# semihkacmaz/CoNFiLD

Measured on AMD Instinct MI355X. Metric: generated fields/sec (256-step sample + CNF decode), Case4 latent, 1/2/4/8 GPU, higher is better.
Workload: dtype f32

## Files before the change

### confild_amd/csrc/unet_kernels.hip

```cpp
#include <algorithm>
#include <cstdlib>

#include "unet_kernels.hpp"

namespace cfd {

__global__ __launch_bounds__(256) void gn_partial_kernel(GnArgs a) {
    const int chunk = blockIdx.x;
    const int64_t b = blockIdx.y;
    const int Ctot = a.Ctot, cq = Ctot / 4, cpg = Ctot / 32;
    const int HW = a.HW;
    const int p0 = (int)((int64_t)HW * chunk / a.nchunks), p1 = (int)((int64_t)HW * (chunk + 1) / a.nchunks);
    const int rows = 256 / cq;
    const int q = threadIdx.x % cq, r0 = threadIdx.x / cq;
    __shared__ double red[2][1024];
    if (r0 < rows) {
        double s[4] = {0, 0, 0, 0}, s2[4] = {0, 0, 0, 0};
        const int c0 = 4 * q;
        for (int p = p0 + r0; p < p1; p += rows) {
            const int64_t pix = b * HW + p;
            const f4 v = c0 < a.C1 ? *(const f4*)(a.src1 + pix * a.C1 + c0)
                                   : *(const f4*)(a.src2 + pix * a.C2 + (c0 - a.C1));
#pragma unroll
            for (int j = 0; j < 4; ++j) {
// ... 1311 lines not shown
            __builtin_amdgcn_global_load_lds((const void*)(src + lane),
                                             (__attribute__((address_space(3))) void*)&ring[stage][piece * 64], 16, 0, 0);
        }
    };
    const int nall = T32 / 32, per = (nall + kcs - 1) / kcs;
    const int blk0 = kc_i * per, nblk = min(per, nall - blk0);
#pragma unroll
    for (int i = 0; i < NS - 1; ++i)
        if (i < nblk) issue(32 * (blk0 + i), i);

    h8v qh[NJ], ql[NJ];
    {
        const int tq = min(q0 + li, T - 1);
#pragma unroll
        for (int j = 0; j < NJ; ++j) {
            const float* qp = base + (int64_t)tq * C3 + 32 * j + 8 * g;
            float v[8];
#pragma unroll
            for (int t = 0; t < 8; ++t) v[t] = qp[t] * a.scale;
            split8_f16(v, qh[j], ql[j]);
        }
    }
    f4 O[ND];
#pragma unroll
    for (int d = 0; d < ND; ++d) O[d] = f4{0.f, 0.f, 0.f, 0.f};
    float mrun = -INFINITY, lrun = 0.f;

    for (int ib = 0; ib < nblk; ++ib) {
        const int kb = 32 * (blk0 + ib), stage = ib % NS;
        if (NS == 3 && ib + 1 < nblk)
            __builtin_amdgcn_s_waitcnt(vmcnt_wait(PPW));
        else
            __builtin_amdgcn_s_waitcnt(vmcnt_wait(0));
        __builtin_amdgcn_s_barrier();
        if (ib + NS - 1 < nblk) issue(kb + 32 * (NS - 1), (ib + NS - 1) % NS);
        if (!active) continue;
        const h8v* kl8 = &ring[stage][lane];
        f4 st[2];
#pragma unroll
        for (int u = 0; u < 2; ++u) {
            st[u] = f4{0.f, 0.f, 0.f, 0.f};
#pragma unroll
            for (int j = 0; j < NJ; ++j) {
                const h8v kh = kl8[((u * NJ + j) * 2) * 64], kl = kl8[((u * NJ + j) * 2 + 1) * 64];
                st[u] = __builtin_amdgcn_mfma_f32_16x16x32_f16(kl, qh[j], st[u], 0, 0, 0);
                st[u] = __builtin_amdgcn_mfma_f32_16x16x32_f16(kh, ql[j], st[u], 0, 0, 0);
                st[u] = __builtin_amdgcn_mfma_f32_16x16x32_f16(kh, qh[j], st[u], 0, 0, 0);
            }
        }
        float mx = -INFINITY;
        if (kb + 32 > T) {
#pragma unroll
            for (int u = 0; u < 2; ++u)
#pragma unroll
                for (int r = 0; r < 4; ++r)
                    if (kb + 16 * u + 4 * g + r >= T) st[u][r] = -INFINITY;
        }
#pragma unroll
        for (int u = 0; u < 2; ++u)
#pragma unroll
            for (int r = 0; r < 4; ++r) mx = fmaxf(mx, st[u][r]);
        mx = fmaxf(mx, __shfl_xor(mx, 16));
        mx = fmaxf(mx, __shfl_xor(mx, 32));
        const float mnew = fmaxf(mrun, mx);
        const float alpha = __builtin_amdgcn_exp2f(mrun - mnew);
        float p[8], ps = 0.f;
#pragma unroll
        for (int u = 0; u < 2; ++u)
#pragma unroll
            for (int r = 0; r < 4; ++r) {
                p[4 * u + r] = __builtin_amdgcn_exp2f(st[u][r] - mnew);
                ps += p[4 * u + r];
            }
        ps += __shfl_xor(ps, 16);
        ps += __shfl_xor(ps, 32);
        lrun = lrun * alpha + ps;
        mrun = mnew;
#pragma unroll
        for (int d = 0; d < ND; ++d) O[d] = O[d] * alpha;
        h8v ph, pl;
        split8_f16(p, ph, pl);
        const h8v* vl8 = &ring[stage][KP * 64 + lane];
#pragma unroll
        for (int d = 0; d < ND; ++d) {
            const h8v vh = vl8[(2 * d) * 64], vl = vl8[(2 * d + 1) * 64];
            O[d] = __builtin_amdgcn_mfma_f32_16x16x32_f16(vl, ph, O[d], 0, 0, 0);
            O[d] = __builtin_amdgcn_mfma_f32_16x16x32_f16(vh, pl, O[d], 0, 0, 0);
            O[d] = __builtin_amdgcn_mfma_f32_16x16x32_f16(vh, ph, O[d], 0, 0, 0);
        }
    }
    if (!active) return;
    const int tq = q0 + li;
    if constexpr (SPLIT) {
        if (tq < T) {
            const int64_t row = ((int64_t)kc_i * (gridDim.z / kcs) + b) * heads + h;
            float* op = a.part + (row * T + tq) * CH;
#pragma unroll
            for (int d = 0; d < ND; ++d) *(f4*)(op + 16 * d + 4 * g) = O[d];
            if (g == 0) {
                float* ml = a.part + (int64_t)kcs * (gridDim.z / kcs) * heads * T * CH;
                *(float2*)(ml + 2 * (row * T + tq)) = float2{mrun, lrun};
            }
        }
        return;
    }
    if (a.lse && g == 0 && tq < T)
        a.lse[((int64_t)b * gridDim.y + h) * T + tq] = (mrun + log2f(lrun)) * 0.69314718055994530942f;
    if (tq < T) {
        float* op = a.out + (b * (int64_t)T + tq) * a.C + (int64_t)h * CH;
        const float inv = 1.0f / lrun;
#pragma unroll
        for (int d = 0; d < ND; ++d) {
            f4 v = O[d] * inv;
            *(f4*)(op + 16 * d + 4 * g) = v;
        }
    }
}

template <int CH>
__global__ __launch_bounds__(256) void attn_combine_kernel(AttnArgs a, int heads, int B) {
    constexpr int Q = CH / 4;
    const int64_t i = (int64_t)blockIdx.x * blockDim.x + threadIdx.x;
    const int64_t rows = (int64_t)B * heads * a.T;
    if (i >= rows * Q) return;
    const int d4 = (int)(i % Q);
    const int64_t r = i / Q;
    const int kc = a.kc;
    const float* ml = a.part + (int64_t)kc * rows * CH;
    float M = -INFINITY;
    for (int c = 0; c < kc; ++c) M = fmaxf(M, ml[2 * (c * rows + r)]);
    float L = 0.f;
    f4 o = {0.f, 0.f, 0.f, 0.f};
    for (int c = 0; c < kc; ++c) {
        const float w = __builtin_amdgcn_exp2f(ml[2 * (c * rows + r)] - M);
        L += w * ml[2 * (c * rows + r) + 1];
        o += w * *(const f4*)(a.part + (c * rows + r) * CH + 4 * d4);
    }
    const int tq = (int)(r % a.T);
    const int64_t bh = r / a.T;
    const int h = (int)(bh % heads);
    const int64_t b = bh / heads;
    *(f4*)(a.out + (b * (int64_t)a.T + tq) * a.C + (int64_t)h * CH + 4 * d4) = o * (1.0f / L);
    if (a.lse && d4 == 0) a.lse[bh * a.T + tq] = (M + log2f(L)) * 0.69314718055994530942f;
}

__global__ void temb_kernel(const int64_t* __restrict__ t, const float* __restrict__ freqs, float* __restrict__ out,
                            int dim) {
    const int b = blockIdx.x;
    const int half = dim / 2;
    const float tf = (float)t[b];
    for (int i = threadIdx.x; i < dim; i += blockDim.x) {
        float v = 0.f;
        if (i < half) {
            v = cosf(tf * freqs[i]);
        } else if (i < 2 * half) {
            v = sinf(tf * freqs[i - half]);
        }
        out[(int64_t)b * dim + i] = v;
    }
}

template <int KW>
__global__ __launch_bounds__(256) void linear_kernel(const float* __restrict__ x, const float* __restrict__ W,
                                                     const float* __restrict__ bias, float* __restrict__ y, int B,
                                                     int K, int N, int act) {
    constexpr int BC = 8;
    extern __shared__ __attribute__((aligned(16))) float xs[];
    const int lane = threadIdx.x & 63;
    const int n = blockIdx.x * 4 + (threadIdx.x >> 6);
    const bool live = n < N;
    CFD_DASSERT(K <= 256 * KW && K % 4 == 0);
    f4 w[KW];
#pragma unroll
    for (int i = 0; i < KW; ++i) {
        const int k = 4 * (lane + 64 * i);
        w[i] = live && k < K ? *(const f4*)(W + (int64_t)n * K + k) : f4{0.f, 0.f, 0.f, 0.f};
    }
    const float bn = live ? bias[n] : 0.f;
    for (int b0 = 0; b0 < B; b0 += BC) {
        const int nb = min(BC, B - b0);
        __syncthreads();
        for (int i = threadIdx.x; i < nb * K; i += 256) {
            const float v = x[(int64_t)b0 * K + i];
            xs[i] = act ? silu_f(v) : v;
        }
        __syncthreads();
        if (!live) continue;
        for (int bb = 0; bb < nb; ++bb) {
            float s = 0.f;
#pragma unroll
            for (int i = 0; i < KW; ++i) {
                const int k = 4 * (lane + 64 * i);
                if (k < K) {
                    const f4 v = *(const f4*)(xs + bb * K + k);
                    s = fmaf(w[i][0], v[0], s);
                    s = fmaf(w[i][1], v[1], s);
                    s = fmaf(w[i][2], v[2], s);
                    s = fmaf(w[i][3], v[3], s);
                }
            }
            for (int o = 32; o > 0; o >>= 1) s += __shfl_xor(s, o);
            if (lane == 0) y[(int64_t)(b0 + bb) * N + n] = s + bn;
        }
    }
}

int gn_chunks(int HW) {
    const int64_t small = std::min<int64_t>(64, HW / 16);
    return (int)std::max<int64_t>(1, std::min<int64_t>(kGnMaxChunks, std::max<int64_t>(HW / 64, small)));
}

static unsigned long long* g_stamps = nullptr;
void stamps_set(unsigned long long* buf) { g_stamps = buf; }
unsigned long long* stamps_buf() { return g_stamps; }
static int g_seq = 0;

static int env_int(const char* name, int dflt) {
    const char* e = getenv(name);
    return e ? atoi(e) : dflt;
}

bool gn2_applies(const GnArgs& a) {
    const int pb = a.plan_b > 0 ? a.plan_b : 8;
    return (int64_t)a.HW * 8 >= (int64_t)4096 * pb && a.Ctot % 4 == 0 && a.C1 % 4 == 0 && a.C2 % 4 == 0 &&
           a.Ctot <= 1024;
}

static int gn_reg_ipt(const GnArgs& a) {
    return a.Ctot % 128 == 0 ? (int)ceil_div(a.HW, 512 / (a.Ctot / 128)) : 0;
}

bool gn_takes_splitk(const GnArgs& a, int B) {
    (void)B;
    if (gn2_applies(a)) return a.C1 % 4 == 0;
    if (a.Ctot % 128 != 0 || a.C1 % 4 != 0) return false;
    return gn_reg_ipt(a) <= 16;
}

void launch_gn(const GnArgs& a0, int B, hipStream_t st) {
    CFD_REQUIRE(a0.Ctot % 32 == 0 && a0.C1 % 4 == 0 && a0.C2 % 4 == 0 && a0.Ctot <= 1024, CFD_ESHAPE,
                "GroupNorm32 needs channels % 32 == 0 (<= 1024)");
    GnArgs a = a0;
    a.nchunks = gn_chunks(a.HW);
    a.B = B;
    a.stamps = g_stamps;
    a.seq = g_seq++;
    CFD_REQUIRE(!a.kpart || gn_takes_splitk(a, B), CFD_ESTATE, "internal: split-K source on a GroupNorm path without it");
    if (gn2_applies(a)) {
        CFD_REQUIRE(!a.kpart || a.kx, CFD_ESTATE, "internal: gn2 needs the split-K sum's destination");
        a.nchunks = gn2_chunks(a.HW, a.plan_b);
        if (gn2_threads(a.nchunks) == 1024) {
            hipLaunchKernelGGL(gn2_stats_kernel<1024>, dim3(a.nchunks, B), dim3(1024), 0, st, a);
            check_launch("gn2_stats_kernel");
            hipLaunchKernelGGL(gn2_apply_kernel<1024>, dim3(a.nchunks, B), dim3(1024), 0, st, a);
        } else {
            hipLaunchKernelGGL(gn2_stats_kernel<256>, dim3(a.nchunks, B), dim3(256), 0, st, a);
            check_launch("gn2_stats_kernel");
            hipLaunchKernelGGL(gn2_apply_kernel<256>, dim3(a.nchunks, B), dim3(256), 0, st, a);
        }
        check_launch("gn2_apply_kernel");
        return;
    }
    const int ipt = gn_reg_ipt(a);
    if (ipt > 0 && ipt <= 32) {
        const dim3 grid((unsigned)(32 * B));
        const int nq = a.Ctot / 128, r256 = 256 / nq, i256 = (a.HW + r256 - 1) / r256;
        if (i256 <= 4) {
            if (i256 <= 1)
                hipLaunchKernelGGL((gn_fused_reg_kernel<1, 256>), grid, dim3(256), 0, st, a);
            else if (i256 <= 2)
                hipLaunchKernelGGL((gn_fused_reg_kernel<2, 256>), grid, dim3(256), 0, st, a);
            else
                hipLaunchKernelGGL((gn_fused_reg_kernel<4, 256>), grid, dim3(256), 0, st, a);
            check_launch("gn_fused_reg_kernel");
            return;
        }
        if (ipt <= 4)
            hipLaunchKernelGGL((gn_fused_reg_kernel<2, 1024>), grid, dim3(1024), 0, st, a);
        else if (ipt <= 8)
            hipLaunchKernelGGL((gn_fused_reg_kernel<4, 1024>), grid, dim3(1024), 0, st, a);
        else if (ipt <= 16)
            hipLaunchKernelGGL((gn_fused_reg_kernel<8, 1024>), grid, dim3(1024), 0, st, a);
        else
            hipLaunchKernelGGL(gn_fused_reg_kernel<32>, grid, dim3(512), 0, st, a);
        check_launch("gn_fused_reg_kernel");
        return;
    }
    hipLaunchKernelGGL(gn_partial_kernel, dim3(a.nchunks, B), dim3(256), 0, st, a);
    check_launch("gn_partial_kernel");
    hipLaunchKernelGGL(gn_finalize_kernel, dim3(B), dim3(1024), 0, st, a);
    check_launch("gn_finalize_kernel");
    const int64_t nq = (int64_t)B * a.HW * a.Ctot / 4;
    hipLaunchKernelGGL(gn_apply_kernel, dim3((unsigned)std::min<int64_t>(4096, ceil_div(nq, 256))), dim3(256), 0, st, a);
    check_launch("gn_apply_kernel");
}


static int even_splits(int nch, int splits) {
    if (splits <= 1) return 1;
    const int per = (nch + splits - 1) / splits;
    return (nch + per - 1) / per;
}

ConvPlan plan_conv(const ConvArgs& a, size_t part_cap_floats) {
    const int plan_b = a.plan_b > 0 ? a.plan_b : 8;
    ConvPlan p;
    const int64_t mn = (int64_t)plan_b * a.Hout * a.Wout;
    p.bn = a.Cout >= 128 ? 128 : 64;
    auto tiles = [&](int bm) { return ceil_div(mn, bm) * ceil_div(a.Cout, p.bn); };
    p.bm = 64;
    int wg_per_tile = 1;
    if (p.bn == 128) {
        p.bm = 128;
        p.nw = 8;
        wg_per_tile = 2;
    }
    const int nkt = a.K / 32;
    p.splits = 1;
    while (tiles(p.bm) * wg_per_tile * p.splits < 768 && nkt / (p.splits * 2) >= 4 && p.splits < 16)
        p.splits *= 2;
    if (a.ks == 1 && !a.tmode && tiles(p.bm) >= 128) p.splits = 1;
    while (p.splits > 1 && (size_t)p.splits * mn * a.Cout > part_cap_floats) p.splits /= 2;
    if (a.wlo && a.ks == 3 && a.stride == 1 && !a.tmode && a.Ctot <= 128 && (int64_t)a.Hout * a.Wout >= 36864)
        return p;
    const int64_t srows = mn / ((int64_t)a.Hout * a.Wout) * a.Hin * a.Win;
    const bool fits32 = srows < (1 << 23) && srows * std::max(a.C1, a.C2) * 4 < (1ll << 30) &&
                        (int64_t)a.Cout * a.K * 2 < (1ll << 31);
    auto halo_splits = [&](int64_t t) {
        const int nch = a.Ctot / 32;
        int sp = 1;
        while (t * sp < 256 && sp * 2 <= nch && sp < 16) sp *= 2;
        while (sp > 1 && (size_t)sp * mn * a.Cout > part_cap_floats) sp /= 2;
        return even_splits(nch, sp);
    };
    if (a.wbf && !a.wlo && !a.tmode && a.ks == 3 && a.stride == 1 && a.Cout >= 128 && fits32 && conv_h_tw(a) > 0) {
        ConvPlan q;
        q.kx = 22;
        q.bm = 256;
        q.bn = 128;
        q.nw = 8;
        q.splits = halo_splits(ceil_div(mn, 256) * ceil_div(a.Cout, 128));
        return q;
    }
    if (a.wbf && a.wlo && !a.tmode && a.ks == 3 && a.stride == 1 && a.Cout >= 128 && fits32) {
        ConvPlan q;
        if (conv_h_tw(a) > 0) {
            q.kx = 20;
            q.bm = 256;
            q.bn = 128;
            q.nw = 8;
            q.splits = halo_splits(ceil_div(mn, 256) * ceil_div(a.Cout, 128));
            return q;
        }
        q.kx = mn >= 2048 ? 2 : 1;
        q.bm = q.kx == 2 ? 256 : 128;
        q.bn = 128;
        q.nw = q.kx == 2 ? 8 : 4;
        const int64_t t = ceil_div(mn, q.bm) * ceil_div(a.Cout, q.bn);
        q.splits = 1;
        while (t * q.splits < 256 && nkt / (q.splits * 2) >= 4 && q.splits < 32) q.splits *= 2;
        while (q.splits > 1 && (size_t)q.splits * mn * a.Cout > part_cap_floats) q.splits /= 2;
        return q;
    }
    return p;
}

int smalln_below() {
    const int v = env_int("CFD_CONV_SMALLN", 1);
    return v == 1 ? 128 : std::max(v, 0);
}

template <bool TMODE, int MODE, bool BUFA>
static void launch_conv_tiles_(const ConvArgs& a, const ConvPlan& p, dim3 grid, hipStream_t st) {
    if constexpr (MODE != 0 && BUFA) {
        static const int smalln = smalln_below();
        if (!TMODE && p.nw == 8 && p.bm == 128 && p.bn == 128 && (int64_t)grid.x * grid.y * grid.z < smalln &&
            a.Cout % 64 == 0) {
            const dim3 g64(grid.x, (unsigned)ceil_div(a.Cout, 64), grid.z);
            hipLaunchKernelGGL((conv_gemm_kernel<128, 64, false, MODE, 8, true>), g64, dim3(512), 0, st, a);
            return;
        }
        if (p.nw == 8 && p.bm == 128 && p.bn == 128 && p.pf == 2) {
            hipLaunchKernelGGL((conv_gemm_kernel<128, 128, TMODE, MODE, 8, true, 2>), grid, dim3(512), 0, st, a);
            return;
        }
        if (p.nw == 8 && p.bm == 128 && p.bn == 128 && p.pf == 3) {
            hipLaunchKernelGGL((conv_gemm_kernel<128, 128, TMODE, MODE, 8, true, 3>), grid, dim3(512), 0, st, a);
            return;
        }
    }
    if (p.nw == 8 && p.bm == 128 && p.bn == 128)
        hipLaunchKernelGGL((conv_gemm_kernel<128, 128, TMODE, MODE, 8, BUFA>), grid, dim3(512), 0, st, a);
    else if (p.bm == 128 && p.bn == 128)
        hipLaunchKernelGGL((conv_gemm_kernel<128, 128, TMODE, MODE, 4, BUFA>), grid, dim3(256), 0, st, a);
    else if (p.bm == 64 && p.bn == 128)
        hipLaunchKernelGGL((conv_gemm_kernel<64, 128, TMODE, MODE, 4, BUFA>), grid, dim3(256), 0, st, a);
    else if (p.bm == 128 && p.bn == 64)
        hipLaunchKernelGGL((conv_gemm_kernel<128, 64, TMODE, MODE, 4, BUFA>), grid, dim3(256), 0, st, a);
    else
        hipLaunchKernelGGL((conv_gemm_kernel<64, 64, TMODE, MODE, 4, BUFA>), grid, dim3(256), 0, st, a);
}

template <bool TMODE, int MODE>
static void launch_conv_tiles(const ConvArgs& a, const ConvPlan& p, dim3 grid, hipStream_t st) {
    if (a.bufaddr) return launch_conv_tiles_<TMODE, MODE, true>(a, p, grid, st);
    launch_conv_tiles_<TMODE, MODE, false>(a, p, grid, st);
}

void launch_splitk_reduce(const ConvArgs& a, int splits, hipStream_t st) {
    const int64_t total4 = (int64_t)a.M * a.Cout / 4;
    hipLaunchKernelGGL(splitk_reduce_kernel, dim3((unsigned)ceil_div(total4, 256)), dim3(256), 0, st, a, splits);
    check_launch("splitk_reduce_kernel");
}

static bool conv_x_falls_back(const ConvArgs& a) {
    static const int force_k1s = env_int("CFD_CONV_FORCE_K1S", 0);
    const int64_t srows = (int64_t)a.Hin * a.Win * (a.M / (a.Hout * a.Wout));
    return force_k1s || !(srows < (1 << 24) && a.M < (1 << 24) && srows * std::max(a.C1, a.C2) * 4 < (1ll << 31));
}

bool conv_runs_k1hb(const ConvArgs& a, const ConvPlan& p) { return p.kx == 22 && !conv_x_falls_back(a); }

bool conv_kv_pack_ok(const ConvArgs& a, const ConvPlan& p, int T) {
    static const int ldsepi = env_int("CFD_CONV_LDSEPI", 1);
    return ldsepi && p.kx < 0 && p.splits == 1 && a.wbf && !a.tmode && a.ks == 1 && a.bias &&
           !a.emb && !a.res && a.Cout % 8 == 0 && a.emb_stride % 4 == 0 && T % 32 == 0 && a.M % T == 0;
}

int launch_conv(const ConvArgs& a, const ConvPlan& p0, hipStream_t st, bool defer) {
    ConvPlan p = p0;
    if (p.kx >= 0 && conv_x_falls_back(a)) {
        p.kx = -1;
        p.bm = p.bn = 128;
        p.nw = 8;
    }
    CFD_REQUIRE(!a.src_bf16 || p.kx == 22, CFD_ESTATE, "internal: a bf16 convolution source needs the K1hb kernel");
    static const int pf = env_int("CFD_CONV_PF", 2);
    if (p.kx < 0) p.pf = pf >= 1 && pf <= 3 ? pf : 1;
    CFD_REQUIRE(a.Ctot % 32 == 0 && a.C1 % 4 == 0 && a.C2 % 4 == 0, CFD_ESHAPE, "conv_gemm needs channels % 32 == 0");
    CFD_REQUIRE(a.K == a.ks * a.ks * a.Ctot, CFD_ESHAPE, "conv K mismatch");
    CFD_REQUIRE(p.splits == 1 || (a.part && a.Cout % 4 == 0), CFD_ESTATE, "split-K needs a partial buffer");
    CFD_REQUIRE(!a.tmode || ((a.stride == 1 || a.stride == 2) && !a.up), CFD_ESHAPE, "transposed conv: stride 1|2");
    const dim3 grid((unsigned)ceil_div(a.M, p.bm), (unsigned)ceil_div(a.Cout, p.bn), p.splits);
    CFD_REQUIRE(!(a.tmode && a.wbf && !a.wlo), CFD_ESTATE, "bf16 input-gradient convolutions are not built");
    static const int xcd = env_int("CFD_CONV_XCD", 4);
    static const int ldsepi = env_int("CFD_CONV_LDSEPI", 1);
    ConvArgs b = a;
    b.stamps = g_stamps;
    b.seq = g_seq++;
    b.ldsepi = ldsepi && a.Cout % 4 == 0 && a.emb_stride % 4 == 0;
    const int xo = xcd == 4 ? (a.wbf && !a.wlo ? 1 : 3) : xcd;
    b.xcd = xo == 3 ? ((int64_t)a.Hout * a.Wout <= 256 ? 2 : 1) : xo < 0 || xo > 2 ? 1 : xo;
    {
        const int64_t srows = (int64_t)a.Hin * a.Win * (a.M / (a.Hout * a.Wout));
        const int64_t wes = (a.wbf || a.wlo) ? 2 : 4;
        b.bufaddr = a.ks * a.ks <= 9 && srows < (1 << 24) && a.M < (1 << 24) &&
                    srows * std::max(a.C1, a.C2) * 4 < (1ll << 31) && (int64_t)a.Cout * a.K * wes < (1ll << 31);
    }
    const ConvArgs& a_ = b;
    if (p.kx >= 0) {
        launch_conv_x(a_, p.kx, p.splits, st);
        if (p.splits > 1 && !defer) launch_splitk_reduce(a, p.splits, st);
        return p.splits;
    }
    if (a.tmode && a.wlo)
        launch_conv_tiles<true, 2>(a_, p, grid, st);
    else if (a.tmode)
        launch_conv_tiles<true, 0>(a_, p, grid, st);
    else if (a.wbf && a.wlo)
        launch_conv_tiles<false, 2>(a_, p, grid, st);
    else if (a.wbf)
        launch_conv_tiles<false, 1>(a_, p, grid, st);
    else
        launch_conv_tiles<false, 0>(a_, p, grid, st);
    check_launch("conv_gemm_kernel");
    if (p.splits > 1 && !defer) launch_splitk_reduce(a, p.splits, st);
    return p.splits;
}

void launch_conv_in(const ConvArgs& a, hipStream_t st) {
    if (a.Cout % 4 == 0 && a.C1 <= 4 && (size_t)9 * a.C1 * a.Cout * 4 <= 64 * 1024) {
        const int64_t n = (int64_t)a.M * (a.Cout / 4);
        hipLaunchKernelGGL(conv_in_vec_kernel, dim3((unsigned)std::min<int64_t>(2048, ceil_div(n, 256))), dim3(256),
                           sizeof(float) * 9 * a.C1 * a.Cout, st, a);
        check_launch("conv_in_vec_kernel");
        return;
    }
    const int64_t n = (int64_t)a.M * a.Cout;
    hipLaunchKernelGGL(conv_in_kernel, dim3((unsigned)ceil_div(n, 256)), dim3(256), 0, st, a);
    check_launch("conv_in_kernel");
}

void launch_conv_out(const ConvArgs& a, hipStream_t st) {
    CFD_REQUIRE(a.Cout <= 4, CFD_ESHAPE, "out_channels must be <= 4");
    const int LP = a.Ctot / 4;
    if (a.Ctot % 4 == 0 && a.C1 == a.Ctot && LP >= 1 && LP <= 64 && (LP & (LP - 1)) == 0 &&
        (size_t)a.Cout * a.K * 4 <= 64 * 1024) {
        const int64_t waves = ceil_div(a.M, 64 / LP);
        hipLaunchKernelGGL(conv_out_vec_kernel, dim3((unsigned)std::min<int64_t>(8192, ceil_div(waves, 4))), dim3(256),
                           sizeof(float) * a.Cout * a.K, st, a, LP);
        check_launch("conv_out_vec_kernel");
        return;
    }
    hipLaunchKernelGGL(conv_out_kernel, dim3((unsigned)ceil_div(a.M, 4)), dim3(256), 0, st, a);
    check_launch("conv_out_kernel");
}

void launch_attention(const AttnArgs& a, int CH, int heads, int B, hipStream_t st) {
    const dim3 grid((unsigned)ceil_div(a.T, 64), heads, B);
    switch (CH) {
        case 16: hipLaunchKernelGGL(attention_kernel<16>, grid, dim3(256), 0, st, a); break;
        case 32: hipLaunchKernelGGL(attention_kernel<32>, grid, dim3(256), 0, st, a); break;
        case 64: hipLaunchKernelGGL(attention_kernel<64>, grid, dim3(256), 0, st, a); break;
        case 128: hipLaunchKernelGGL(attention_kernel<128>, grid, dim3(256), 0, st, a); break;
        default: throw Error{CFD_ESHAPE, "attention head channels must be 16, 32, 64 or 128"};
    }
    check_launch("attention_kernel");
}

size_t attention_split_floats(int T, int C) { return (size_t)(T + 31) / 32 * 32 * C * 2; }

int64_t attention_split_voff(int T, int CH, int heads, int B) {
    const int T32 = (T + 31) / 32 * 32;
    return (int64_t)B * heads * (T32 / 16) * (CH / 32) * 128;
}

int attention_kv_chunks(int T, int heads, int plan_b) {
    const int nblk = (T + 31) / 32;
    const int64_t wgs = (int64_t)plan_b * heads * ceil_div(T, 64);
    int kc = 1;
    while (kc * 4 <= nblk && wgs * kc * 2 <= 256) kc *= 2;
    return kc;
}

size_t attention_part_floats(int T, int C, int CH, int plan_b) {
    const int heads = C / CH, kc = attention_kv_chunks(T, heads, plan_b);
    return kc == 1 ? 0 : (size_t)kc * T * (C + 2 * heads);
}

void launch_attention_split(const AttnArgs& a, int CH, int heads, int B, int plan_b, float* kvws, hipStream_t st,
                            bool packed) {
    CFD_REQUIRE(CH == 32 || CH == 64 || CH == 128, CFD_ESHAPE, "split attention needs head channels 32, 64 or 128");
    const int T32 = (a.T + 31) / 32 * 32;
    h8v* kf = (h8v*)kvws;
    h8v* vf = kf + attention_split_voff(a.T, CH, heads, B);
    if (!packed) {
        const int64_t slots = (int64_t)B * heads * ((T32 / 16) * (CH / 32) * 64 + (T32 / 32) * (CH / 16) * 64);
        hipLaunchKernelGGL(attn_kv_split_kernel, dim3((unsigned)ceil_div(slots, 256)), dim3(256), 0, st, a, CH, heads,
                           B, kf, vf);
        check_launch("attn_kv_split_kernel");
    }
    const int kc = attention_kv_chunks(a.T, heads, plan_b);
    if (kc > 1) {
        CFD_REQUIRE(a.part, CFD_ESTATE, "internal: key-chunked attention without a partial buffer");
        AttnArgs a2 = a;
        a2.kc = kc;
        a2.xcdmap = 0;
        const dim3 grid((unsigned)ceil_div(a.T, 64), heads, B * kc);
        switch (CH) {
            case 32: hipLaunchKernelGGL((attention_dma_kernel<32, 4, 3, true>), grid, dim3(256), 0, st, a2, kf, vf); break;
            case 64: hipLaunchKernelGGL((attention_dma_kernel<64, 4, 3, true>), grid, dim3(256), 0, st, a2, kf, vf); break;
            default: hipLaunchKernelGGL((attention_dma_kernel<128, 4, 3, true>), grid, dim3(256), 0, st, a2, kf, vf); break;
        }
        check_launch("attention_dma_kernel (key chunks)");
        const int64_t n = (int64_t)B * heads * a.T * (CH / 4);
        const dim3 g2((unsigned)ceil_div(n, 256));
        switch (CH) {
            case 32: hipLaunchKernelGGL(attn_combine_kernel<32>, g2, dim3(256), 0, st, a2, heads, B); break;
            case 64: hipLaunchKernelGGL(attn_combine_kernel<64>, g2, dim3(256), 0, st, a2, heads, B); break;
            default: hipLaunchKernelGGL(attn_combine_kernel<128>, g2, dim3(256), 0, st, a2, heads, B); break;
        }
        check_launch("attn_combine_kernel");
        return;
    }
    static const int xcdmap = env_int("CFD_ATTN_XCD", 1);
    AttnArgs a2 = a;
    a2.xcdmap = xcdmap && (heads * B) % 8 == 0 ? 1 : 0;
    const int w8 = a.T >= 512 && (int64_t)B * heads * ceil_div(a.T, 128) >= 256;
    const dim3 grid((unsigned)ceil_div(a.T, w8 ? 128 : 64), heads, B);
    const dim3 blk(w8 ? 512 : 256);
    switch (CH * 2 + w8) {
        case 64: hipLaunchKernelGGL((attention_dma_kernel<32, 4>), grid, blk, 0, st, a2, kf, vf); break;
        case 65: hipLaunchKernelGGL((attention_dma_kernel<32, 8>), grid, blk, 0, st, a2, kf, vf); break;
        case 128: hipLaunchKernelGGL((attention_dma_kernel<64, 4>), grid, blk, 0, st, a2, kf, vf); break;
        case 129: hipLaunchKernelGGL((attention_dma_kernel<64, 8>), grid, blk, 0, st, a2, kf, vf); break;
        case 256: hipLaunchKernelGGL((attention_dma_kernel<128, 4>), grid, blk, 0, st, a2, kf, vf); break;
        default: hipLaunchKernelGGL((attention_dma_kernel<128, 8>), grid, blk, 0, st, a2, kf, vf); break;
    }
    check_launch("attention_dma_kernel");
}

void launch_temb(const int64_t* t, const float* freqs, float* out, int dim, int B, hipStream_t st) {
    hipLaunchKernelGGL(temb_kernel, dim3(B), dim3(128), 0, st, t, freqs, out, dim);
    check_launch("temb_kernel");
}

void launch_linear(const float* x, const float* W, const float* bias, float* y, int B, int K, int N, int act,
                   hipStream_t st) {
    CFD_REQUIRE(K % 4 == 0 && K <= 2048, CFD_ESHAPE, "linear: K must be a multiple of 4, at most 2048");
    const dim3 g((unsigned)ceil_div(N, 4));
    const size_t lds = sizeof(float) * 8 * K;
    if (K <= 256) hipLaunchKernelGGL(linear_kernel<1>, g, dim3(256), lds, st, x, W, bias, y, B, K, N, act);
    else if (K <= 512) hipLaunchKernelGGL(linear_kernel<2>, g, dim3(256), lds, st, x, W, bias, y, B, K, N, act);
    else if (K <= 1024) hipLaunchKernelGGL(linear_kernel<4>, g, dim3(256), lds, st, x, W, bias, y, B, K, N, act);
    else hipLaunchKernelGGL(linear_kernel<8>, g, dim3(256), lds, st, x, W, bias, y, B, K, N, act);
    check_launch("linear_kernel");
}

}

extern "C" int cfd_stamps_set(void* buf) {
#ifdef CFD_STAMPS
    cfd::stamps_set((unsigned long long*)buf);
    return CFD_OK;
#else
    (void)buf;
    cfd::set_error("cfd_stamps_set: not a CFD_STAMPS build (make STAMPS=1)");
    return CFD_ESTATE;
#endif
}
```

### confild_amd/csrc/unet_kernels.hpp

```cpp
#pragma once
#include "common.hpp"

namespace cfd {

struct GnArgs {
    const float* src1;
    const float* src2;
    const float* gamma;
    const float* beta;
    double* part;
    float* ss;
    float* out;
    float* stats;
    int C1, C2, Ctot, HW;
    float eps;
    int silu;
    int nchunks;
    int B;
    const float* kpart;
    const float* kbias;
    const float* kemb;
    const float* kres;
    float* kx;
    int ksplits, kemb_stride;
    unsigned long long* stamps;
    int seq;
    int out_bf16;
    unsigned* amax_out;
    int plan_b;
};

struct ConvArgs {
    const float* src1;
    const float* src2;
    const float* w;
    const void* wbf;
    const void* wlo;
    float acc_scale;
    const float* bias;
    const float* emb;
    const float* res;
    float* out;
    float* part;
    int C1, C2, Ctot;
    int Hin, Win, Hout, Wout;
    int stride, ks, pad, up;
    int tmode;
    int Cout;
    int emb_stride;
    int M, K;
    int xcd;
    int bufaddr;
    int ldsepi;
    int* nonfinite;
    int src_bf16;
    void* kvf;
    int64_t kv_voff;
    int kv_ch, kv_heads, kv_T;
    float kv_scale;
    unsigned long long* stamps;
    int seq;
    int plan_b;
};
void stamps_set(unsigned long long* buf);
unsigned long long* stamps_buf();

struct AttnArgs {
    const float* qkv;
    float* out;
    int T, C;
    float scale;
    float* lse;
    int xcdmap;
    int kc;
    float* part;
};

struct GnbArgs {
    const float* x1;
    const float* x2;
    const float* dz;
    const float* ss;
    const float* stats;
    const float* gamma;
    const float* addsrc;
    float* out1;
    float* out2;
    int acc1, acc2;
    double* part;
    float* fin;
    float* ppart;
    unsigned* amax_out;
    int C1, C2, Ctot, HW, silu, nchunks, B;
    int plan_b;
};

struct AttnBwdArgs {
    const float* qkv;
    const float* o;
    const float* dout;
    const float* lse;
    float* dd;
    float* dqkv;
    int T, C;
    float scale;
    h8v* packs;
    float* amax;
    int heads, xcdmap;
};

struct ConvPlan {
    int bm = 128, bn = 128, splits = 1;
    int nw = 4;
    int kx = -1;
    int pf = 1;
};

constexpr int kGnMaxChunks = 512;
int gn_chunks(int HW);
constexpr int kGn2BigHW = 16384, kGn2BigChunks = 256;
static_assert(kGn2BigChunks <= kGnMaxChunks, "gn2 partials live in the kGnMaxChunks slab");
int gn2_chunks(int HW, int plan_b);
inline int gn2_threads(int nchunks) { return nchunks > 64 ? 1024 : 256; }
void launch_gn(const GnArgs& a, int B, hipStream_t st);
bool gn_takes_splitk(const GnArgs& a, int B);
bool gn2_applies(const GnArgs& a);
ConvPlan plan_conv(const ConvArgs& a, size_t part_cap_floats);
int launch_conv(const ConvArgs& a, const ConvPlan& p, hipStream_t st, bool defer = false);
void launch_splitk_reduce(const ConvArgs& a, int splits, hipStream_t st);
__device__ __forceinline__ void xcd_tile(int order, int& bx, int& by, int& bz) {
    bx = blockIdx.x;
    by = blockIdx.y;
    bz = blockIdx.z;
    if (!order) return;
    const unsigned gx = gridDim.x, gy = gridDim.y, gz = gridDim.z;
    const unsigned T = gx * gy * gz, L = blockIdx.x + gx * (blockIdx.y + gy * blockIdx.z);
    const unsigned q = T >> 3, r = T & 7, x = L & 7, sl = L >> 3;
    const unsigned Lp = x < r ? x * (q + 1) + sl : r * (q + 1) + (x - r) * q + sl;
    if (order == 2) {
        bx = Lp % gx;
        bz = (Lp / gx) % gz;
        by = Lp / (gx * gz);
    } else {
        bz = Lp % gz;
        by = (Lp / gz) % gy;
        bx = Lp / (gz * gy);
    }
}
int launch_conv_x(const ConvArgs& a, int variant, int splits, hipStream_t st);
int conv_h_tw(const ConvArgs& a);
int smalln_below();
bool conv_runs_k1hb(const ConvArgs& a, const ConvPlan& p);
void launch_conv_in(const ConvArgs& a, hipStream_t st);
void launch_conv_out(const ConvArgs& a, hipStream_t st);
void launch_attention(const AttnArgs& a, int CH, int heads, int B, hipStream_t st);
size_t attention_split_floats(int T, int C);
int attention_kv_chunks(int T, int heads, int plan_b);
size_t attention_part_floats(int T, int C, int CH, int plan_b);
void launch_attention_split(const AttnArgs& a, int CH, int heads, int B, int plan_b, float* kvws, hipStream_t st,
                            bool packed);
int64_t attention_split_voff(int T, int CH, int heads, int B);
bool conv_kv_pack_ok(const ConvArgs& a, const ConvPlan& p, int T);
int launch_gn_bwd(const GnbArgs& a, int B, hipStream_t st);
void launch_attention_bwd(const AttnBwdArgs& a, int CH, int heads, int B, hipStream_t st);
size_t attention_bwd_split_floats(int T, int C);
bool attention_bwd_split_ok(int T, int CH);
void launch_attention_bwd_split(const AttnBwdArgs& a, int CH, int heads, int B, float* ws, hipStream_t st);
void launch_add(float* y, const float* x, int64_t n, hipStream_t st);
void launch_temb(const int64_t* t, const float* freqs, float* out, int dim, int B, hipStream_t st);
void launch_linear(const float* x, const float* W, const float* bias, float* y, int B, int K, int N, int act,
                   hipStream_t st);


__device__ __forceinline__ float kln2(float scale) { return scale * 1.44269504088896340736f; }
__device__ __forceinline__ void split8_f16(const float (&v)[8], h8v& hi, h8v& lo) {
#pragma clang fp contract(off)
#pragma unroll
    for (int t = 0; t < 8; ++t) {
        hi[t] = (_Float16)v[t];
        lo[t] = (_Float16)(v[t] - (float)hi[t]);
    }
}
constexpr int vmcnt_wait(int n) { return (n & 15) | (7 << 4) | (15 << 8) | (((n >> 4) & 3) << 14); }
}
```

Before: 3.752.

## Add dedicated pointwise split-f16 MFMA conv kernel with tile-size variants

Adds a new kernel for 1x1 stride-1 forward convolutions that use split-f16 weights (hi/lo). It loads f32 activations through buffer loads and splits them into f16 hi/lo with fma_mix instructions. It then runs three f16 MFMAs per tile pair out of a double-buffered swizzled LDS layout with register prefetch. The planner routes eligible pointwise convs to one of three tile variants chosen by tile count, and the new kernel also takes the fused KV-pack epilogue. The aim is to replace the generic im2col-style conv GEMM path and its split-K for these layers, at the cost of more code paths and no split-K for small-tile cases.

```diff
diff --git a/confild_amd/csrc/conv_p.hip b/confild_amd/csrc/conv_p.hip
--- /dev/null
+++ b/confild_amd/csrc/conv_p.hip
@@ -0,0 +1,276 @@
+#include <algorithm>
+
+#include "unet_kernels.hpp"
+
+namespace cfd {
+
+__device__ __forceinline__ int pswz(int row, int chunk) { return row * 64 + ((chunk + 2 * ((row >> 2) & 1)) & 3) * 16; }
+
+__device__ __forceinline__ void split4_mix_p(const f4& x, uint2& hi, uint2& lo) {
+    typedef _Float16 h2_ __attribute__((ext_vector_type(2)));
+    typedef float f2_ __attribute__((ext_vector_type(2)));
+    hi.x = __builtin_bit_cast(unsigned, __builtin_convertvector((f2_){x[0], x[1]}, h2_));
+    hi.y = __builtin_bit_cast(unsigned, __builtin_convertvector((f2_){x[2], x[3]}, h2_));
+    asm("v_fma_mixlo_f16 %0, %1, 1.0, -%2 op_sel_hi:[0,0,1]" : "=&v"(lo.x) : "v"(x[0]), "v"(hi.x));
+    asm("v_fma_mixhi_f16 %0, %1, 1.0, -%2 op_sel:[0,0,1] op_sel_hi:[0,0,1]" : "+v"(lo.x) : "v"(x[1]), "v"(hi.x));
+    asm("v_fma_mixlo_f16 %0, %1, 1.0, -%2 op_sel_hi:[0,0,1]" : "=&v"(lo.y) : "v"(x[2]), "v"(hi.y));
+    asm("v_fma_mixhi_f16 %0, %1, 1.0, -%2 op_sel:[0,0,1] op_sel_hi:[0,0,1]" : "+v"(lo.y) : "v"(x[3]), "v"(hi.y));
+}
+
+template <int BM, int BN, int NW, int PF>
+__global__ __launch_bounds__(64 * NW, NW == 4 ? 2 : 1) void conv_p_kernel(ConvArgs a) {
+    constexpr int NT = 64 * NW;
+    constexpr int WM = BM / (NW / 2), WN = BN / 2;
+    constexpr int TM = WM / 16, TN = WN / 16;
+    constexpr int RPP = NT / 8;
+    constexpr int AIT = BM / RPP, BIT = BN / RPP;
+    static_assert(TM >= 1 && TN >= 1 && AIT >= 1 && BIT >= 1 && BM % RPP == 0 && BN % RPP == 0, "tile");
+    constexpr int APL = BM * 64, BPL = BN * 64;
+    constexpr int STAGE = 2 * APL + 2 * BPL;
+    static_assert(BM * BN * 4 <= 2 * STAGE && BM % 32 == 0 && BM * BN / 4 % NT == 0, "epilogue tile");
+    __shared__ __attribute__((aligned(16))) char lds[2 * STAGE];
+
+    CFD_STAMP(a.stamps, 3, a.seq, 0);
+    const int tid = threadIdx.x, lane = tid & 63, wave = tid >> 6;
+    const int wm = wave >> 1, wn = wave & 1;
+    int bx, by, bz;
+    xcd_tile(a.xcd, bx, by, bz);
+    const int m0 = bx * BM, n0 = by * BN;
+    const int kq = tid & 7, rsub = tid >> 3;
+
+    const __amdgpu_buffer_rsrc_t rs1 = __builtin_amdgcn_make_buffer_rsrc((void*)a.src1, 0, a.M * a.C1 * 4, 0x00020000);
+    const __amdgpu_buffer_rsrc_t rs2 = __builtin_amdgcn_make_buffer_rsrc(
+        (void*)(a.src2 ? a.src2 : a.src1), 0, a.src2 ? a.M * a.C2 * 4 : 0, 0x00020000);
+    const __amdgpu_buffer_rsrc_t rwh = __builtin_amdgcn_make_buffer_rsrc((void*)a.wbf, 0, a.Cout * a.K * 2, 0x00020000);
+    const __amdgpu_buffer_rsrc_t rwl = __builtin_amdgcn_make_buffer_rsrc((void*)a.wlo, 0, a.Cout * a.K * 2, 0x00020000);
+    unsigned a_off1[AIT], a_off2[AIT], b_off[BIT];
+#pragma unroll
+    for (int it = 0; it < AIT; ++it) {
+        const int m = m0 + rsub + it * RPP;
+        a_off1[it] = m < a.M ? (unsigned)(m * a.C1 + 4 * kq) * 4u : 0x80000000u;
+        a_off2[it] = m < a.M ? (unsigned)(m * a.C2 + 4 * kq) * 4u : 0x80000000u;
+    }
+#pragma unroll
+    for (int it = 0; it < BIT; ++it) {
+        const int n = n0 + rsub + it * RPP;
+        b_off[it] = n < a.Cout ? (unsigned)(n * a.K + 4 * kq) * 2u : 0x80000000u;
+    }
+    const int nkt = a.K / 32;
+
+    f4 ra[PF][AIT];
+    uint2 rbh[PF][BIT], rbl[PF][BIT];
+    auto load_tile = [&](int kt, int sl) {
+        const int cb = __builtin_amdgcn_readfirstlane(kt * 32);
+        const bool second = cb >= a.C1;
+        const __amdgpu_buffer_rsrc_t rsa = second ? rs2 : rs1;
+        const int sa = (second ? cb - a.C1 : cb) * 4;
+        CFD_DASSERT(cb + 32 <= a.K && (second ? cb - a.C1 + 32 <= a.C2 : cb + 32 <= a.C1));
+#pragma unroll
+        for (int it = 0; it < AIT; ++it) {
+            CFD_DASSERT(m0 + rsub + it * RPP >= a.M || (second ? a_off2[it] : a_off1[it]) + sa + 16 <=
+                                                           (unsigned)a.M * (second ? a.C2 : a.C1) * 4u);
+            ra[sl][it] = __builtin_bit_cast(
+                f4, __builtin_amdgcn_raw_buffer_load_b128(rsa, second ? a_off2[it] : a_off1[it], sa, 0));
+        }
+#pragma unroll
+        for (int it = 0; it < BIT; ++it) {
+            rbh[sl][it] = __builtin_bit_cast(uint2, __builtin_amdgcn_raw_buffer_load_b64(rwh, b_off[it], cb * 2, 0));
+            rbl[sl][it] = __builtin_bit_cast(uint2, __builtin_amdgcn_raw_buffer_load_b64(rwl, b_off[it], cb * 2, 0));
+        }
+    };
+    auto store_tile = [&](int buf, int sl) {
+        char* st = lds + buf * STAGE;
+#pragma unroll
+        for (int it = 0; it < AIT; ++it) {
+            uint2 hv, lv;
+            split4_mix_p(ra[sl][it], hv, lv);
+            const int off = pswz(rsub + it * RPP, kq >> 1) + (kq & 1) * 8;
+            CFD_DASSERT(off >= 0 && off + 8 <= APL);
+            *(uint2*)(st + off) = hv;
+            *(uint2*)(st + APL + off) = lv;
+        }
+#pragma unroll
+        for (int it = 0; it < BIT; ++it) {
+            const int off = pswz(rsub + it * RPP, kq >> 1) + (kq & 1) * 8;
+            CFD_DASSERT(off >= 0 && off + 8 <= BPL);
+            *(uint2*)(st + 2 * APL + off) = rbh[sl][it];
+            *(uint2*)(st + 2 * APL + BPL + off) = rbl[sl][it];
+        }
+    };
+
+    f4 acc[TM][TN];
+#pragma unroll
+    for (int i = 0; i < TM; ++i)
+#pragma unroll
+        for (int j = 0; j < TN; ++j) acc[i][j] = f4{0.f, 0.f, 0.f, 0.f};
+    const int g = lane >> 4, li = lane & 15;
+    auto compute = [&](int cur) {
+        const char* st = lds + cur * STAGE;
+        h8v fah[TM], fal[TM], fbh[TN], fbl[TN];
+#pragma unroll
+        for (int i = 0; i < TM; ++i) {
+            const int off = pswz(wm * WM + 16 * i + li, g);
+            CFD_DASSERT(off + 16 <= APL);
+            fah[i] = *(const h8v*)(st + off);
+            fal[i] = *(const h8v*)(st + APL + off);
+        }
+#pragma unroll
+        for (int j = 0; j < TN; ++j) {
+            const int off = pswz(wn * WN + 16 * j + li, g);
+            CFD_DASSERT(off + 16 <= BPL);
+            fbh[j] = *(const h8v*)(st + 2 * APL + off);
+            fbl[j] = *(const h8v*)(st + 2 * APL + BPL + off);
+        }
+#pragma unroll
+        for (int i = 0; i < TM; ++i)
+#pragma unroll
+            for (int j = 0; j < TN; ++j) {
+                acc[i][j] = __builtin_amdgcn_mfma_f32_16x16x32_f16(fal[i], fbh[j], acc[i][j], 0, 0, 0);
+                acc[i][j] = __builtin_amdgcn_mfma_f32_16x16x32_f16(fah[i], fbl[j], acc[i][j], 0, 0, 0);
+                acc[i][j] = __builtin_amdgcn_mfma_f32_16x16x32_f16(fah[i], fbh[j], acc[i][j], 0, 0, 0);
+            }
+    };
+
+#pragma unroll
+    for (int p = 0; p < PF; ++p) load_tile(min(p, nkt - 1), p);
+    store_tile(0, 0);
+    __syncthreads();
+    CFD_STAMP(a.stamps, 3, a.seq, 2);
+    auto step = [&](int k, int j) {
+        load_tile(min(k + PF, nkt - 1), j);
+        compute(k & 1);
+        store_tile((k & 1) ^ 1, (j + 1) % PF);
+        __syncthreads();
+        __builtin_amdgcn_sched_barrier(0);
+    };
+    int k = 0;
+    for (; k + PF <= nkt; k += PF) {
+#pragma unroll
+        for (int j = 0; j < PF; ++j) step(k + j, j);
+    }
+#pragma unroll
+    for (int j = 0; j < PF - 1; ++j)
+        if (k + j < nkt) step(k + j, j);
+    CFD_STAMP(a.stamps, 3, a.seq, 3);
+
+    float* tile = (float*)lds;
+    auto sw = [](int row, int col) { return row * BN + (col ^ (((row >> 2) & 3) << 4)); };
+    const int g4 = 4 * g;
+#pragma unroll
+    for (int i = 0; i < TM; ++i)
+#pragma unroll
+        for (int j = 0; j < TN; ++j) {
+            acc[i][j] *= a.acc_scale;
+#pragma unroll
+            for (int r = 0; r < 4; ++r) {
+                const int o = sw(wm * WM + 16 * i + g4 + r, wn * WN + 16 * j + li);
+                CFD_DASSERT(o >= 0 && o < BM * BN);
+                tile[o] = acc[i][j][r];
+            }
+        }
+    __syncthreads();
+    constexpr int NV = BM * BN / 4 / NT;
+#pragma unroll
+    for (int v = 0; v < NV; ++v) {
+        const int idx = tid + v * NT;
+        const int row = idx / (BN / 4), c4 = (idx - row * (BN / 4)) * 4;
+        const int m = m0 + row, n = n0 + c4;
+        if (m >= a.M || n >= a.Cout) continue;
+        f4 val = *(const f4*)&tile[sw(row, c4)];
+        const int64_t o = (int64_t)m * a.Cout + n;
+        if (a.bias) val = val + *(const f4*)(a.bias + n);
+        if (a.res) val = *(const f4*)(a.res + o) + val;
+        *(f4*)(a.out + o) = val;
+    }
+    if (a.kvf) {
+        const int CH = a.kv_ch, C3 = 3 * CH, T = a.kv_T, nj = CH >> 5, nd = CH >> 4;
+        const float ks = kln2(a.kv_scale);
+        const float rc3 = 1.0f / (float)C3, rT = 1.0f / (float)T;
+        h8v* kf = (h8v*)a.kvf;
+        h8v* vf = kf + a.kv_voff;
+        for (int it = tid; it < BM * (BN / 8); it += NT) {
+            const int row = it / (BN / 8), c8 = (it - row * (BN / 8)) * 8;
+            const int m = m0 + row, n = n0 + c8;
+            if (m >= a.M || n >= a.Cout) continue;
+            const int hh = fdiv24(n, C3, rc3), o = n - hh * C3;
+            if (o < CH || o >= 2 * CH) continue;
+            const int b = fdiv24(m, T, rT);
+            const int kc = o - CH, key = m - b * T;
+            f4 v0 = *(const f4*)&tile[sw(row, c8)], v1 = *(const f4*)&tile[sw(row, c8 + 4)];
+            v0 = v0 + *(const f4*)(a.bias + n);
+            v1 = v1 + *(const f4*)(a.bias + n + 4);
+            float v[8];
+#pragma unroll
+            for (int t = 0; t < 4; ++t) {
+                v[t] = v0[t] * ks;
+                v[t + 4] = v1[t] * ks;
+            }
+            h8v hi, lo;
+            split8_f16(v, hi, lo);
+            const int64_t bh = (int64_t)b * a.kv_heads + hh;
+            h8v* dst = kf + ((bh * (T >> 4) + (key >> 4)) * nj + (kc >> 5)) * 128 + ((kc & 31) >> 3) * 16 + (key & 15);
+            CFD_DASSERT(b * T + key < a.M && hh < a.kv_heads && kc < CH);
+            dst[0] = hi;
+            dst[64] = lo;
+        }
+        for (int it = tid; it < (BM / 32) * 4 * BN; it += NT) {
+            const int col = it % BN, r2 = it / BN, gg = r2 & 3, blk = r2 >> 2;
+            const int n = n0 + col, mb = m0 + 32 * blk;
+            if (n >= a.Cout || mb >= a.M) continue;
+            const int hh = fdiv24(n, C3, rc3), o = n - hh * C3;
+            if (o < 2 * CH) continue;
+            const int b = fdiv24(mb, T, rT);
+            const int vc = o - 2 * CH, kb = (mb - b * T) >> 5;
+            const float bn = a.bias[n];
+            float v[8];
+#pragma unroll
+            for (int t = 0; t < 8; ++t) v[t] = tile[sw(32 * blk + (t < 4 ? 4 * gg + t : 12 + 4 * gg + t), col)] + bn;
+            h8v hi, lo;
+            split8_f16(v, hi, lo);
+            const int64_t bh = (int64_t)b * a.kv_heads + hh;
+            h8v* dst = vf + ((bh * (T >> 5) + kb) * nd + (vc >> 4)) * 128 + gg * 16 + (vc & 15);
+            CFD_DASSERT(mb + 32 <= a.M && hh < a.kv_heads && vc < CH);
+            dst[0] = hi;
+            dst[64] = lo;
+        }
+    }
+#ifdef CFD_STAMPS
+    __builtin_amdgcn_s_waitcnt(0);
+#endif
+    CFD_STAMP(a.stamps, 3, a.seq, 4);
+}
+
+bool conv_p_applies(const ConvArgs& a) {
+#ifdef CFD_NO_K1P
+    return false;
+#else
+    return a.wbf && a.wlo && !a.tmode && a.ks == 1 && a.stride == 1 && !a.up && !a.src_bf16 && !a.emb &&
+           a.C1 % 32 == 0 && a.C2 % 32 == 0 && a.Ctot >= 32 && (a.C2 == 0 || a.src2) && a.Cout % 4 == 0 &&
+           a.Hin == a.Hout && a.Win == a.Wout;
+#endif
+}
+
+void conv_p_tile(int variant, int& bm, int& bn, int& nw) {
+    bm = variant == 40 ? 128 : variant == 41 ? 64 : 32;
+    bn = variant == 40 ? 128 : 64;
+    nw = variant == 40 ? 8 : 4;
+}
+
+void launch_conv_p(const ConvArgs& a, int variant, hipStream_t st) {
+    CFD_REQUIRE(conv_p_applies(a) && a.K == a.Ctot, CFD_ESTATE, "internal: K1p takes pointwise split-f16 forward convolutions");
+    CFD_REQUIRE((int64_t)a.M * std::max(a.C1, a.C2) * 4 < (1ll << 31) && (int64_t)a.Cout * a.K * 2 < (1ll << 31) &&
+                    a.M < (1 << 24),
+                CFD_ESTATE, "internal: K1p needs 32-bit operand offsets");
+    int bm, bn, nw;
+    conv_p_tile(variant, bm, bn, nw);
+    const dim3 grid((unsigned)ceil_div(a.M, bm), (unsigned)ceil_div(a.Cout, bn), 1);
+    switch (variant) {
+        case 40: hipLaunchKernelGGL((conv_p_kernel<128, 128, 8, 2>), grid, dim3(512), 0, st, a); break;
+        case 41: hipLaunchKernelGGL((conv_p_kernel<64, 64, 4, 3>), grid, dim3(256), 0, st, a); break;
+        case 42: hipLaunchKernelGGL((conv_p_kernel<32, 64, 4, 4>), grid, dim3(256), 0, st, a); break;
+        default: throw Error{CFD_ESTATE, "internal: unknown K1p variant"};
+    }
+    check_launch("conv_p_kernel");
+}
+
+}
diff --git a/confild_amd/csrc/unet_kernels.hip b/confild_amd/csrc/unet_kernels.hip
--- a/confild_amd/csrc/unet_kernels.hip
+++ b/confild_amd/csrc/unet_kernels.hip
@@ -1637,6 +1637,8 @@
     return (nch + per - 1) / per;
 }
 
+constexpr int64_t kK1pMin128 = 144, kK1pMin64 = 192;
+
 ConvPlan plan_conv(const ConvArgs& a, size_t part_cap_floats) {
     const int plan_b = a.plan_b > 0 ? a.plan_b : 8;
     ConvPlan p;
@@ -1656,6 +1658,14 @@
         p.splits *= 2;
     if (a.ks == 1 && !a.tmode && tiles(p.bm) >= 128) p.splits = 1;
     while (p.splits > 1 && (size_t)p.splits * mn * a.Cout > part_cap_floats) p.splits /= 2;
+    if (conv_p_applies(a) && !(ceil_div(mn, 32) * ceil_div(a.Cout, 64) < 32 && a.K >= 1024)) {
+        ConvPlan q;
+        const int64_t t128 = ceil_div(mn, 128) * ceil_div(a.Cout, 128), t64 = ceil_div(mn, 64) * ceil_div(a.Cout, 64);
+        q.kx = t128 >= kK1pMin128 ? 40 : t64 >= kK1pMin64 ? 41 : 42;
+        conv_p_tile(q.kx, q.bm, q.bn, q.nw);
+        q.splits = 1;
+        return q;
+    }
     if (a.wlo && a.ks == 3 && a.stride == 1 && !a.tmode && a.Ctot <= 128 && (int64_t)a.Hout * a.Wout >= 36864)
         return p;
     const int64_t srows = mn / ((int64_t)a.Hout * a.Wout) * a.Hin * a.Win;
@@ -1754,17 +1764,21 @@
     return force_k1s || !(srows < (1 << 24) && a.M < (1 << 24) && srows * std::max(a.C1, a.C2) * 4 < (1ll << 31));
 }
 
+static bool conv_p_falls_back(const ConvArgs& a) {
+    return !conv_p_applies(a) || (int64_t)a.Cout * a.K * 2 >= (1ll << 31);
+}
+
 bool conv_runs_k1hb(const ConvArgs& a, const ConvPlan& p) { return p.kx == 22 && !conv_x_falls_back(a); }
 
 bool conv_kv_pack_ok(const ConvArgs& a, const ConvPlan& p, int T) {
     static const int ldsepi = env_int("CFD_CONV_LDSEPI", 1);
-    return ldsepi && p.kx < 0 && p.splits == 1 && a.wbf && !a.tmode && a.ks == 1 && a.bias &&
+    return ldsepi && (p.kx < 0 || p.kx >= 40) && p.splits == 1 && a.wbf && !a.tmode && a.ks == 1 && a.bias &&
            !a.emb && !a.res && a.Cout % 8 == 0 && a.emb_stride % 4 == 0 && T % 32 == 0 && a.M % T == 0;
 }
 
 int launch_conv(const ConvArgs& a, const ConvPlan& p0, hipStream_t st, bool defer) {
     ConvPlan p = p0;
-    if (p.kx >= 0 && conv_x_falls_back(a)) {
+    if (p.kx >= 0 && (conv_x_falls_back(a) || (p.kx >= 40 && conv_p_falls_back(a)))) {
         p.kx = -1;
         p.bm = p.bn = 128;
         p.nw = 8;
@@ -1793,6 +1807,11 @@
                     srows * std::max(a.C1, a.C2) * 4 < (1ll << 31) && (int64_t)a.Cout * a.K * wes < (1ll << 31);
     }
     const ConvArgs& a_ = b;
+    if (p.kx >= 40) {
+        CFD_REQUIRE(p.splits == 1, CFD_ESTATE, "internal: K1p does not split over K");
+        launch_conv_p(a_, p.kx, st);
+        return 1;
+    }
     if (p.kx >= 0) {
         launch_conv_x(a_, p.kx, p.splits, st);
         if (p.splits > 1 && !defer) launch_splitk_reduce(a, p.splits, st);
diff --git a/confild_amd/csrc/unet_kernels.hpp b/confild_amd/csrc/unet_kernels.hpp
--- a/confild_amd/csrc/unet_kernels.hpp
+++ b/confild_amd/csrc/unet_kernels.hpp
@@ -149,6 +149,9 @@
 }
 int launch_conv_x(const ConvArgs& a, int variant, int splits, hipStream_t st);
 int conv_h_tw(const ConvArgs& a);
+bool conv_p_applies(const ConvArgs& a);
+void conv_p_tile(int variant, int& bm, int& bn, int& nw);
+void launch_conv_p(const ConvArgs& a, int variant, hipStream_t st);
 int smalln_below();
 bool conv_runs_k1hb(const ConvArgs& a, const ConvPlan& p);
 void launch_conv_in(const ConvArgs& a, hipStream_t st);
```

Measured after the change: 3.795 (median of 6 runs). +1.2%, better.
